# antonilo/unsupervised_detection

Hardware: NVIDIA H100
Metric: frame-pairs/sec adversarial train step 256x448 (higher is better)
Workload: dtype bf16

## Files before the change

unsupervised_detection_b200/csrc/conv_igemm.cu:

```cuda
#include "ptx.cuh"
#include "../../include/cis_b200.h"
#include "common.cuh"
#include <cuda.h>
#include <stdlib.h>
#include <string.h>


namespace cis {

#ifdef CIS_TRACE
__device__ unsigned long long* g_trace = nullptr;
__device__ int g_trace_cap = 0;
#define CIS_TRACE_AT(slot)                                                                                         \
  do {                                                                                                             \
    if (g_trace && blockIdx.x == 0 && blockIdx.y == 0 && blockIdx.z == 0 && (slot) < g_trace_cap) g_trace[(slot)] = clock64(); \
  } while (0)
#else
#define CIS_TRACE_AT(slot) ((void)0)
#endif

static constexpr int kBM = 128;
static constexpr int kBK = 64;
static constexpr int kAStage = kBM * 128;
static constexpr int kThreads = 256;
template <int BN, int NWG> struct HaloCfg {
  static_assert(NWG == 1 || (NWG == 2 && BN >= 64), "two MMA warpgroups only for BN >= 64");
  static constexpr int kMmaWarp = (NWG == 1 && BN >= 64) ? 8 : 4;
  static constexpr int kThreads = (kMmaWarp + 4 * NWG) * 32;
  static constexpr int kEpiWarps = NWG == 1 ? kMmaWarp : kThreads / 32;
  static constexpr int kEpiParts = NWG == 1 ? (BN >= 64 ? 2 : 1) : BN / 32;
  static constexpr int kMaxMT = (128 / BN) < 4 ? (128 / BN) : 4;
};
static constexpr int kMaxAccCols = 128;
static constexpr int kGProducers = 256;
static constexpr int kGThreads = 384;

struct SrcS {
  const __nv_bfloat16* ptr;
  int pitch, c_off, chunks, n_mod;
};


__device__ __forceinline__ void epi_chunk(const CisConv& p, float (&v)[16], const int cg, const size_t dpix) {
  if (p.bias) {
#pragma unroll
    for (int e = 0; e < 16; ++e) v[e] += __ldg(p.bias + cg + e);
  }
  if (p.add_pre && cg < p.out_ch) {
    const uint4* a = reinterpret_cast<const uint4*>(reinterpret_cast<const __nv_bfloat16*>(p.add_pre) + dpix * p.add_pre_pitch +
                                                    p.add_pre_coff + cg);
    const int nv = (p.out_ch - cg >= 16) ? 2 : 1;
    for (int h2 = 0; h2 < nv; ++h2) {
      const uint4 u = __ldg(a + h2);
      const uint32_t w4[4] = {u.x, u.y, u.z, u.w};
#pragma unroll
      for (int e = 0; e < 4; ++e) {
        v[h2 * 8 + 2 * e] += bf16lo(w4[e]);
        v[h2 * 8 + 2 * e + 1] += bf16hi(w4[e]);
      }
    }
  }
  if (p.addf_pre) {
    for (int e = 0; e < 16 && cg + e < p.outf_ch; ++e) v[e] += __ldg(p.addf_pre + dpix * p.addf_pitch + p.addf_coff + cg + e);
  }
// ... 183 lines not shown
#pragma unroll
    for (int h = 0; h < 4; ++h) t[h] = __ldcg(q0 + (size_t)z * zstride + h * kBM);
#pragma unroll
    for (int h = 0; h < 4; ++h) {
      v[4 * h] += t[h].x; v[4 * h + 1] += t[h].y; v[4 * h + 2] += t[h].z; v[4 * h + 3] += t[h].w;
    }
  }
}
template <int BN, typename DPIX>
__device__ __forceinline__ void cluster_reduce_rows(const CisConv& p, const uint32_t stage, const int S, const int rank, const int tid,
                                                    const int nthreads, const int cbase, DPIX dpix_of) {
  const int rpc = (kBM + S - 1) / S;
  const int r0 = rank * rpc, r1 = min(kBM, r0 + rpc);
  constexpr int G16 = BN / 16;
  for (int it = tid; it < (r1 - r0) * G16; it += nthreads) {
    const int row = r0 + it / G16, c0 = (it % G16) * 16;
    float v[16];
#pragma unroll
    for (int e = 0; e < 16; ++e) v[e] = 0.f;
    for (int q = 0; q < S; ++q) {
      const uint32_t base = dsmem_addr(stage, (uint32_t)q);
#pragma unroll
      for (int h = 0; h < 4; ++h) {
        const float4 t = dsmem_ld4(base + (uint32_t)(((c0 / 4 + h) * kBM + row) * 16));
        v[4 * h] += t.x; v[4 * h + 1] += t.y; v[4 * h + 2] += t.z; v[4 * h + 3] += t.w;
      }
    }
    bool valid;
    const size_t dpix = dpix_of(row, valid);
    if (valid) epi_chunk(p, v, cbase + c0, dpix);
  }
}

template <int BN>
struct FwdCfg {
  static constexpr int kStages = (BN == 128) ? 3 : 4;
  static constexpr int kLag = kStages - 2;
  static constexpr int kBStage = BN * 128;
  static constexpr int kSmem = kStages * (kAStage + kBStage) + 1024;
  static_assert(kStages * (kAStage + kBStage) >= kBM * BN * 4, "the accumulator tile reuses the operand ring");
};

template <int BN>
__global__ void __launch_bounds__(kGThreads) conv_igemm_kernel(const __grid_constant__ CisConv p) {
  using Cfg = FwdCfg<BN>;
  constexpr int S = Cfg::kStages;
  constexpr int kMmaWarp = kGProducers / 32;
  extern __shared__ uint8_t smem_raw[];
  __shared__ uint64_t bars[2 * S + 1];
  __shared__ int s_dh[CIS_MAX_TAPS], s_dw[CIS_MAX_TAPS];
  __shared__ SrcS s_src[CIS_MAX_SRC];

  const uint32_t tile_base = (smem_u32(smem_raw) + 1023u) & ~1023u;
  const uint32_t a_base = tile_base;
  const uint32_t b_base = tile_base + S * kAStage;
  const uint32_t bar_full = smem_u32(&bars[0]);
  const uint32_t bar_empty = smem_u32(&bars[S]);
  const uint32_t bar_accum = smem_u32(&bars[2 * S]);

  const int tid = threadIdx.x;
  const int warp = tid >> 5, lane = tid & 31;
  const int M = p.N * p.OH * p.OW;
  const int m_chunks = [&] {
    int s = 0;
    for (int i = 0; i < p.nsrc; ++i) s += p.src[i].chunks;
    return s;
  }();
  const int nkb_all = p.K_pad / kBK;
  const int nsplit = p.splits > 1 ? p.splits : 1;
  const int kper = (nkb_all + nsplit - 1) / nsplit;
  const int kb_lo = blockIdx.z * kper;
  const int nkb = min(kper, nkb_all - kb_lo);
  const int ny = blockIdx.y;
  __shared__ __align__(16) float s_bias[BN];
  pdl_launch_dependents();

  if (tid < p.ntaps) {
    s_dh[tid] = p.dh[tid];
    s_dw[tid] = p.dw[tid];
  }
  if (tid < p.nsrc) {
    s_src[tid].ptr = reinterpret_cast<const __nv_bfloat16*>(p.src[tid].ptr);
    s_src[tid].pitch = p.src[tid].pitch;
    s_src[tid].c_off = p.src[tid].c_off;
    s_src[tid].chunks = p.src[tid].chunks;
    s_src[tid].n_mod = p.src[tid].n_mod;
  }
  if (tid == kMmaWarp * 32) {
    for (int s = 0; s < S; ++s) {
      mbar_init(bar_full + 8 * s, kGProducers);
      mbar_init(bar_empty + 8 * s, 1);
    }
    mbar_init(bar_accum, 128);
    fence_mbar_init();
  }
  pdl_wait();
  if (tid < BN) s_bias[tid] = p.bias ? p.bias[ny * BN + tid] : 0.f;
  __syncthreads();
  if (tid == 0) CIS_TRACE_AT(0);

  if (warp < kMmaWarp) {
    const int j = tid & 7;
    const int rl = tid >> 3;
    const uint32_t sw_off = (uint32_t)((j ^ (rl & 7)) << 4);
    int hb[4], wb[4], pre[4], prem[4];
    int nm0 = 0;
    for (int i = 0; i < p.nsrc; ++i)
      if (p.src[i].n_mod > 0 && nm0 == 0) nm0 = p.src[i].n_mod;
#pragma unroll
    for (int i = 0; i < 4; ++i) {
      const int g = blockIdx.x * kBM + rl + 32 * i;
      if (g < M) {
        const int ow = g % p.OW;
        const int t = g / p.OW;
        const int oh = t % p.OH;
        const int n = t / p.OH;
        hb[i] = oh * p.sh;
        wb[i] = ow * p.sw;
        pre[i] = (n * p.H + hb[i]) * p.W + wb[i];
        prem[i] = ((nm0 ? n % nm0 : n) * p.H + hb[i]) * p.W + wb[i];
      } else {
        hb[i] = -(1 << 20);
        wb[i] = 0;
        pre[i] = prem[i] = 0;
      }
    }
    const __nv_bfloat16* wrow = reinterpret_cast<const __nv_bfloat16*>(p.wpack) + (size_t)(ny * BN + rl) * p.K_pad + j * 8;
    const int adv_t = 8 / m_chunks, adv_c = 8 - adv_t * m_chunks;
    int t = (kb_lo * 8 + j) / m_chunks, c = (kb_lo * 8 + j) - t * m_chunks;

    for (int kb = 0; kb < nkb; ++kb) {
      const int s = kb % S;
      const uint32_t ph = (uint32_t)((kb / S) & 1);
      mbar_wait(bar_empty + 8 * s, ph ^ 1u);
      const bool kvalid = t < p.ntaps;
      const int tt = kvalid ? t : 0;
      int si = 0, cs = c;
// ... 20 lines not shown
        }
        cp_async16(a_dst + i * 32 * 128, ok ? (const void*)(spc + (size_t)pix * pitch) : (const void*)sp, ok ? 16u : 0u);
      }
      t += adv_t;
      c += adv_c;
      if (c >= m_chunks) {
        c -= m_chunks;
        ++t;
      }
      const uint32_t b_dst = b_base + s * Cfg::kBStage + rl * 128 + sw_off;
      if constexpr (BN >= 32) {
#pragma unroll
        for (int i = 0; i < BN / 32; ++i) cp_async16(b_dst + i * 32 * 128, wrow + (size_t)i * 32 * p.K_pad + (kb_lo + kb) * kBK, 16u);
      } else {
        if (rl < BN) cp_async16(b_dst, wrow + (kb_lo + kb) * kBK, 16u);
      }
      cp_async_commit();
      if (kb >= Cfg::kLag) {
        cp_async_wait<Cfg::kLag>();
        fence_proxy_async();
        mbar_arrive(bar_full + 8 * ((kb - Cfg::kLag) % S));
      }
    }
#pragma unroll
    for (int i = Cfg::kLag - 1; i >= 0; --i) {
      if (nkb - 1 - i < 0) continue;
      if (i == 3) cp_async_wait<3>();
      else if (i == 2) cp_async_wait<2>();
      else if (i == 1) cp_async_wait<1>();
      else cp_async_wait<0>();
      fence_proxy_async();
      mbar_arrive(bar_full + 8 * ((nkb - 1 - i) % S));
    }

    mbar_wait(bar_accum, 0);
    if (tid == 0) CIS_TRACE_AT(2);
    const int qtr = warp & 3, half = warp >> 2;
    const int row = qtr * 32 + lane;
    const int g = blockIdx.x * kBM + row;
    const bool valid = g < M;
    size_t dpix = 0;
    if (valid) {
      const int ow = g % p.OW;
      const int t = g / p.OW;
      const int oh = t % p.OH;
      const int n = t / p.OH;
      dpix = (size_t)(n * p.DH + oh * p.osh + p.oa) * p.DW + ow * p.osw + p.ob;
    }
    const uint32_t t_row = tile_base + (uint32_t)row * 16;
    const int cbase = ny * BN;
    constexpr int kHalf = BN >= 32 ? BN / 2 : BN;
    const int c_lo = half * kHalf, c_hi = (BN >= 32 || half == 0) ? c_lo + kHalf : c_lo;
    if (nsplit > 1 && p.sk_cluster) {
    } else if (nsplit > 1) {
      const int tile_id = blockIdx.x * gridDim.y + ny;
      float* tile0 = p.sk_scratch + (size_t)tile_id * nsplit * kBM * BN;
      splitk_store_partial<BN>(tile0 + (size_t)blockIdx.z * kBM * BN, t_row, row, c_lo, c_hi);
    } else {
      epi_cols<BN>(p, t_row, cbase, dpix, valid, s_bias, c_lo, c_hi);
    }
  } else {
    const int wtid = tid - kMmaWarp * 32;
    float acc[BN];
    const uint32_t dhi = desc_hi(1024);
    constexpr uint32_t a_half = (8 * 1024) >> 4;
    for (int kb = 0; kb < nkb; ++kb) {
      const int s = kb % S;
      mbar_wait(bar_full + 8 * s, (uint32_t)((kb / S) & 1));
      if (wtid == 0) CIS_TRACE_AT(8 + 2 * kb);
      const uint32_t alo = desc_lo(a_base + s * kAStage, 16), blo = desc_lo(b_base + s * Cfg::kBStage, 16);
      wg_fence();
#pragma unroll
      for (int k = 0; k < kBK / 16; ++k) mma128<BN, 0, 0>(acc, alo + 2 * k, dhi, blo + 2 * k, dhi, a_half, (uint32_t)((kb | k) != 0));
      wg_commit();
      wg_wait<1>();
      if (wtid == 0 && kb > 0) mbar_arrive(bar_empty + 8 * ((kb - 1) % S));
      if (wtid == 0) CIS_TRACE_AT(9 + 2 * kb);
    }
    wg_wait<0>();
    acc_store<BN>(acc, tile_base, wtid);
    mbar_arrive(bar_accum);
  }
  if (nsplit > 1 && p.sk_cluster) {
    cluster_sync_all();
    if (warp < kMmaWarp) {
      const int cbase = ny * BN;
      cluster_reduce_rows<BN>(p, tile_base, nsplit, (int)cluster_ctarank(), tid, kGProducers, cbase, [&](int row, bool& valid) -> size_t {
        const int g = blockIdx.x * kBM + row;
        valid = g < M;
        if (!valid) return 0;
        const int ow = g % p.OW;
        const int t = g / p.OW;
        const int oh = t % p.OH;
        const int n = t / p.OH;
        return (size_t)(n * p.DH + oh * p.osh + p.oa) * p.DW + ow * p.osw + p.ob;
      });
    }
    cluster_sync_all();
  }
  if (tid == 0) CIS_TRACE_AT(3);
}


static constexpr int kHaloMaxBStages = 8;
struct HaloMaps {
  CUtensorMap m[CIS_MAX_SRC * 4];
  CUtensorMap w;
  int wrow;
  int16_t wk[2 * CIS_MAX_TAPS];
};
__device__ __forceinline__ void wrow_load(const HaloMaps& maps, const uint32_t dst, const uint32_t bar, const int s0, const int ns, const int n0,
                                          const int BN) {
  for (int s = 0; s < ns; ++s)
// ... 56 lines not shown
    while (ph < p.nph - 1 && t >= p.ph_tap[ph + 1]) ++ph;
  return (uint32_t)(ph * (p.thin / 8)) * plane16 + (uint32_t)(p.dh[t] * Wh + p.dw[t]);
}
__device__ __forceinline__ uint32_t halo_step_off(const CisConv& p, const int t0, const int nt, const int s, const int Wh, const uint32_t plane16) {
  if (!p.thin) return (uint32_t)((p.dh[t0 + s] * Wh + p.dw[t0 + s]) * 8);
  const int ta = p.thin == 8 ? 2 * s : s;
  const uint32_t o0 = halo_tap_off(p, t0 + ta, Wh, plane16);
  if (p.thin == 16) return o0 | (plane16 << 16);
  const uint32_t o1 = ta + 1 < nt ? halo_tap_off(p, t0 + ta + 1, Wh, plane16) : o0;
  return o0 | ((o1 - o0) << 16);
}
template <typename Src>
__device__ __forceinline__ void thin_halo_load(const CisConv& p, const Src* src, const HaloMaps& maps, const uint32_t dst, const uint32_t bar,
                                               const int HP, const int x0, const int y0, const int n) {
  const int nph = p.nph > 1 ? p.nph : 1, npl = p.thin / 8, pb16 = thin_plane_bytes(HP);
  int nld = 0;
  for (int ph = 0; ph < nph; ++ph) nld += nph == 1 || p.ph_tap[ph + 1] > p.ph_tap[ph];
  mbar_expect_tx(bar, (uint32_t)(nld * npl * HP * 16));
  for (int ph = 0; ph < nph; ++ph) {
    if (nph > 1 && p.ph_tap[ph + 1] == p.ph_tap[ph]) continue;
    for (int q = 0; q < npl; ++q) {
      int cq = q, sq = 0;
      while (sq < p.nsrc - 1 && cq >= src[sq].chunks) {
        cq -= src[sq].chunks;
        ++sq;
      }
      const int nm = src[sq].n_mod;
      tma_load_4d(dst + (ph * npl + q) * pb16, &maps.m[sq * nph + ph], bar, cq * 8, x0, y0, nm ? (n % nm) : n);
    }
  }
}

template <int BN, int NWG>
__global__ void __launch_bounds__(HaloCfg<BN, NWG>::kThreads, 1) conv_halo_kernel(const __grid_constant__ CisConv p, const int halo_stage_bytes, const int BS, const int NHS,
                                                        const __grid_constant__ HaloMaps maps, const int use_tma, const int G) {
  using Cfg = HaloCfg<BN, NWG>;
  constexpr int kBStage = BN * 128;
  constexpr int kHMmaWarp_ = Cfg::kMmaWarp, kHThreads_ = Cfg::kThreads;
  extern __shared__ uint8_t smem_raw[];
  __shared__ uint64_t bars[2 * 2 + 2 * kHaloMaxBStages + 1];
  __shared__ uint32_t s_aoff[CIS_MAX_TAPS];
  __shared__ SrcS s_src[CIS_MAX_SRC];

  const int tid = threadIdx.x, warp = tid >> 5, lane = tid & 31;
  const int MT = p.MT, MTC = NWG * MT, d = p.dil;
  const int nph = p.nph > 1 ? p.nph : 1;
  const int Wh = 8 + p.ex, Hh = 16 * MTC + p.ey, HP = Wh * Hh;
  const int thin = p.thin;
  const int nhph = thin ? 1 : nph;
  const uint32_t wstep = thin ? BN * 32 : kBStage;
  const uint32_t stage_bytes = (uint32_t)G * wstep;
  const uint32_t tile_base = (smem_u32(smem_raw) + 1023u) & ~1023u;
  const uint32_t h_base = tile_base;
  const uint32_t b_base = tile_base + NHS * halo_stage_bytes;
  int* pixtab = reinterpret_cast<int*>(smem_raw + (b_base + BS * stage_bytes - smem_u32(smem_raw)));
  const uint32_t bar_hfull = smem_u32(&bars[0]), bar_hempty = smem_u32(&bars[2]);
  const uint32_t bar_bfull = smem_u32(&bars[4]), bar_bempty = smem_u32(&bars[4 + kHaloMaxBStages]);
  const uint32_t bar_accum = smem_u32(&bars[4 + 2 * kHaloMaxBStages]);

  const bool grouped = p.nsub > 1;
  const int tap0 = grouped ? p.sub[blockIdx.z].tap0 : 0, ntaps = grouped ? p.sub[blockIdx.z].ntaps : p.ntaps;
  const int nst = halo_nsteps(thin, ntaps);
  const int hoy = grouped ? p.sub[blockIdx.z].hoy : p.hoy, hox = grouped ? p.sub[blockIdx.z].hox : p.hox;
  const int OHs = grouped ? p.sub[blockIdx.z].OH : p.OH, OWs = grouped ? p.sub[blockIdx.z].OW : p.OW;
  const int oa = grouped ? p.sub[blockIdx.z].oa : p.oa, ob = grouped ? p.sub[blockIdx.z].ob : p.ob;
  const void* const wpack = grouped ? p.sub[blockIdx.z].wpack : p.wpack;
  const int Hp0 = (OHs + d - 1) / d, Wp0 = (OWs + d - 1) / d;
// ... 19 lines not shown
  if (tid < nst) s_aoff[tid] = halo_step_off(p, tap0, ntaps, tid, Wh, (uint32_t)thin_plane_bytes(HP) >> 4);
  if (tid < p.nsrc) {
    s_src[tid].ptr = reinterpret_cast<const __nv_bfloat16*>(p.src[tid].ptr);
    s_src[tid].pitch = p.src[tid].pitch;
    s_src[tid].c_off = p.src[tid].c_off;
    s_src[tid].chunks = p.src[tid].chunks;
    s_src[tid].n_mod = p.src[tid].n_mod;
  }
  for (int q = tid; q < (use_tma ? 0 : HP); q += kHThreads_) {
    const int hy = q / Wh, hx = q - hy * Wh;
    const int gy = ty * 16 * MTC + hy + hoy, gx = tx * 8 + hx + hox;
    const int y = pa + d * gy, x = pb + d * gx;
    pixtab[q] = (gy >= 0 && gx >= 0 && y < p.H && x < p.W) ? (y * p.W + x) : -1;
  }
  if (tid == kHMmaWarp_ * 32) {
    for (int s = 0; s < 2; ++s) {
      mbar_init(bar_hfull + 8 * s, use_tma ? 1 : 96);
      mbar_init(bar_hempty + 8 * s, NWG);
    }
    for (int s = 0; s < BS; ++s) {
      mbar_init(bar_bfull + 8 * s, 1);
      mbar_init(bar_bempty + 8 * s, NWG);
    }
    mbar_init(bar_accum, 128 * NWG);
    fence_mbar_init();
  }
  if (use_tma && tid < p.nsrc) tma_prefetch_desc(&maps.m[tid]);
  pdl_wait();
  if (tid < BN) s_bias[tid] = p.bias ? p.bias[ny * BN + tid] : 0.f;
  __syncthreads();
  if (tid == 0) CIS_TRACE_AT(0);

  if (warp < kHMmaWarp_) {
   if (warp < 4) {
    if (use_tma) {
      if (tid == 0) {
        int hcount = 0;
        for (int vc = 0; vc < nchunks * nhph; ++vc) {
          const int cc = vc / nhph, ph = vc - cc * nhph;
          if (nhph > 1 && p.ph_tap[ph + 1] == p.ph_tap[ph]) continue;
          const int hs = hcount % NHS;
          mbar_wait(bar_hempty + 8 * hs, (uint32_t)(((hcount / NHS) & 1) ^ 1));
          ++hcount;
          int c = (cc_lo + cc) * 8, si = 0;
          while (si < p.nsrc - 1 && c >= s_src[si].chunks) {
            c -= s_src[si].chunks;
            ++si;
          }
          const int nmod = s_src[si].n_mod;
          if (thin) {
            thin_halo_load(p, s_src, maps, h_base + hs * halo_stage_bytes, bar_hfull + 8 * hs, HP, tx * 8 + hox, ty * 16 * MTC + hoy, n);
            continue;
          }
          mbar_expect_tx(bar_hfull + 8 * hs, (uint32_t)(HP * 128));
          tma_load_4d(h_base + hs * halo_stage_bytes, &maps.m[si * nph + ph], bar_hfull + 8 * hs, c * 8, pb + d * (tx * 8 + hox),
                      pa + d * (ty * 16 * MTC + hoy), nmod ? (n % nmod) : n);
        }
      }
      __syncwarp();
    } else if (warp != 2) {
      const int hid = warp == 3 ? tid - 32 : tid;
      const int j = hid & 7, pl = hid >> 3;
      for (int cc = 0; cc < nchunks; ++cc) {
        const int hs = cc % NHS;
        mbar_wait(bar_hempty + 8 * hs, (uint32_t)(((cc / NHS) & 1) ^ 1));
        const int rem = m_chunks - (cc_lo + cc) * 8;
        const int nk16 = rem >= 8 ? 4 : (rem + 1) / 2;
// ... 29 lines not shown
        } else if (cc >= 1) {
          cp_async_wait<1>();
          fence_proxy_async();
          mbar_arrive(bar_hfull + 8 * ((cc - 1) % NHS));
        }
      }
      if (NHS > 1) {
        cp_async_wait<0>();
        fence_proxy_async();
        mbar_arrive(bar_hfull + 8 * ((nchunks - 1) % NHS));
      }
    }
    if (tid == 64) {
      const uint8_t* wt = reinterpret_cast<const uint8_t*>(wpack) + ((size_t)ny * nchunks_all + cc_lo) * nst * wstep;
      int bs = 0;
      uint32_t bph = 1;
      for (int vc = 0; vc < nchunks * nhph; ++vc) {
        const int cc = vc / nhph, ph = vc - cc * nhph;
        const int tlo = nhph > 1 ? p.ph_tap[ph] : 0, thi = nhph > 1 ? p.ph_tap[ph + 1] : nst;
        for (int t0 = tlo; t0 < thi; t0 += G) {
          const uint32_t bytes = (uint32_t)min(G, thi - t0) * wstep;
          mbar_wait(bar_bempty + 8 * bs, bph);
          mbar_expect_tx(bar_bfull + 8 * bs, bytes);
          if (maps.wrow) wrow_load(maps, b_base + bs * stage_bytes, bar_bfull + 8 * bs, t0, min(G, thi - t0), ny * BN, BN);
          else bulk_g2s(b_base + bs * stage_bytes, wt + (size_t)(cc * nst + t0) * wstep, bytes, bar_bfull + 8 * bs);
          if (++bs == BS) {
            bs = 0;
            bph ^= 1u;
          }
        }
      }
    }
    __syncwarp();
   }

  } else {
    const int wg = NWG > 1 ? (warp - kHMmaWarp_) >> 2 : 0;
    const int wtid = tid - (kHMmaWarp_ + 4 * wg) * 32;
    constexpr int MTM = Cfg::kMaxMT;
    float acc[MTM][BN];
    const uint32_t pix = thin ? 16u : 128u;
    const uint32_t ahi = thin ? desc_hi_ns((uint32_t)Wh * pix) : desc_hi((uint32_t)Wh * pix);
    const uint32_t bhi = thin ? desc_hi_ns(maps.wrow ? 128u : 256u) : desc_hi(1024), b_lbo = maps.wrow ? BN * 16u : thin ? 128u : 16u;
    const uint32_t a_mstep = (16u * Wh * pix) >> 4;
    const uint32_t a_half = (8u * Wh * pix) >> 4;
    const uint32_t a_wg = (uint32_t)(wg * MT) * a_mstep;
    int bs = 0, hs = 0, it = 0;
    uint32_t bph = 0, hph = 0;
    bool any = false;
    for (int vc = 0; vc < nchunks * nhph; ++vc) {
      const int cc = vc / nhph, ph = vc - cc * nhph;
      const int tlo = nhph > 1 ? p.ph_tap[ph] : 0, thi = nhph > 1 ? p.ph_tap[ph + 1] : nst;
      if (thi == tlo) continue;
      const int rem = m_chunks - (cc_lo + cc) * 8;
      const int nk16 = rem >= 8 ? 4 : (rem + 1) / 2;
      mbar_wait(bar_hfull + 8 * hs, hph);
      if (vc == 0 && wtid == 0 && wg == 0) CIS_TRACE_AT(1);
      const uint32_t hlo = desc_lo(h_base + hs * halo_stage_bytes, thin ? 0 : 16) + a_wg;
      for (int t0 = tlo; t0 < thi; t0 += G, ++it) {
        const int gt = min(G, thi - t0);
        mbar_wait(bar_bfull + 8 * bs, bph);
        if (wtid == 0 && wg == 0) CIS_TRACE_AT(8 + 2 * it);
        const uint32_t blo = desc_lo(b_base + bs * stage_bytes, b_lbo);
        halo_issue_any<BN, MTM>(nk16, acc, hlo, blo, s_aoff + t0, gt, MT, ahi, bhi, a_mstep, a_half, wstep >> 4, !any);
        if (wtid == 0) {
          mbar_arrive(bar_bempty + 8 * bs);
          if (t0 + G >= thi) mbar_arrive(bar_hempty + 8 * hs);
          if (wg == 0) CIS_TRACE_AT(9 + 2 * it);
        }
        any = true;
        if (++bs == BS) {
          bs = 0;
          bph ^= 1u;
        }
      }
      if (++hs == NHS) {
        hs = 0;
        hph ^= 1u;
      }
    }
    if constexpr (NWG > 1) asm volatile("bar.sync 1, %0;" ::"n"(128 * NWG) : "memory");
#pragma unroll
    for (int m = 0; m < MTM; ++m)
      if (m < MT) acc_store<BN>(acc[m], tile_base + (uint32_t)((wg * MT + m) * BN) * kAccColBytes, wtid);
    mbar_arrive(bar_accum);
  }

  if (warp < Cfg::kEpiWarps) {
    mbar_wait(bar_accum, 0);
    if (tid == 0) CIS_TRACE_AT(2);
    constexpr int kParts = Cfg::kEpiParts, kCols = BN / kParts, kUnits = 4 * kParts;
    const int cbase = ny * BN;
    const int tile_id = blockIdx.x * gridDim.y + ny;
    if (!(nsplit > 1 && p.sk_cluster)) {
#pragma unroll 1
      for (int u = warp; u < MTC * kUnits; u += Cfg::kEpiWarps) {
        const int m = u / kUnits, r = (u & 3) * 32 + lane, c_lo = ((u >> 2) % kParts) * kCols, c_hi = c_lo + kCols;
        const uint32_t t_row = tile_base + (uint32_t)(m * BN) * kAccColBytes + (uint32_t)r * 16;
        if (nsplit > 1) {
          splitk_store_partial<BN>(p.sk_scratch + (((size_t)tile_id * MTC + m) * nsplit + blockIdx.z) * kBM * BN, t_row, r, c_lo, c_hi);
        } else {
          const int gy = ty * 16 * MTC + 16 * m + (r >> 3), gx = tx * 8 + (r & 7);
          const int oy = pa + d * gy, ox = pb + d * gx;
          const bool valid = oy < OHs && ox < OWs;
          const size_t dpix = valid ? ((size_t)(n * p.DH + oy * p.osh + oa) * p.DW + ox * p.osw + ob) : 0;
          epi_cols<BN>(p, t_row, cbase, dpix, valid, s_bias, c_lo, c_hi);
        }
      }
    }
  }
  if (nsplit > 1 && p.sk_cluster) {
    cluster_sync_all();
    if (warp < 4) {
      const int cbase = ny * BN;
      for (int m = 0; m < MTC; ++m)
        cluster_reduce_rows<BN>(p, tile_base + (uint32_t)m * (kBM * BN * 4), nsplit, (int)cluster_ctarank(), tid, 128, cbase,
                                [&](int row, bool& valid) -> size_t {
// ... 699 lines not shown
  cfg.numAttrs = pdl_enabled() ? 1 : 0;
  return cudaLaunchKernelEx(&cfg, kern, KArgs(args)...);
}

template <typename... KArgs, typename... Args>
static cudaError_t launch_pdl_zcluster(void (*kern)(KArgs...), dim3 grid, dim3 block, size_t smem, cudaStream_t st, int cz, Args... args) {
  cudaLaunchConfig_t cfg;
  memset(&cfg, 0, sizeof(cfg));
  cfg.gridDim = grid;
  cfg.blockDim = block;
  cfg.dynamicSmemBytes = smem;
  cfg.stream = st;
  cudaLaunchAttribute attr[2];
  attr[0].id = cudaLaunchAttributeClusterDimension;
  attr[0].val.clusterDim.x = 1;
  attr[0].val.clusterDim.y = 1;
  attr[0].val.clusterDim.z = cz;
  attr[1].id = cudaLaunchAttributeProgrammaticStreamSerialization;
  attr[1].val.programmaticStreamSerializationAllowed = 1;
  cfg.attrs = attr;
  cfg.numAttrs = pdl_enabled() ? 2 : 1;
  return cudaLaunchKernelEx(&cfg, kern, KArgs(args)...);
}

template <int BN>
static cudaError_t launch_splitk_finish(const CisConv* d, dim3 main_grid, cudaStream_t st) {
  constexpr int G = BN / 16;
  constexpr int kBlock = (128 * G < 256) ? 128 * G : 256;
  constexpr int kSub = 128 * G / kBlock;
  const int mt = d->halo ? d->MT * (d->nwg > 1 ? d->nwg : 1) : 1;
  return launch_pdl(splitk_finish_kernel<BN>, dim3(main_grid.x, main_grid.y, mt * kSub), dim3(kBlock), 0, st, *d);
}

template <int BN>
static int launch_fwd(const CisConv* d, cudaStream_t st) {
  using Cfg = FwdCfg<BN>;
  static bool attr_set = false;
  if (!attr_set) {
    cudaError_t e = cudaFuncSetAttribute(conv_igemm_kernel<BN>, cudaFuncAttributeMaxDynamicSharedMemorySize, Cfg::kSmem);
    if (e != cudaSuccess) return cis_set_cuda_error(e, "cudaFuncSetAttribute(conv_igemm)");
    attr_set = true;
  }
  const int M = d->N * d->OH * d->OW;
  int splits = d->splits > 1 ? d->splits : 1;
  if (splits > 1) {
    const int nkb = d->K_pad / kBK, per = (nkb + splits - 1) / splits;
    if ((!d->sk_scratch && !d->sk_cluster) || d->sk_counters || (splits - 1) * per >= nkb || (d->sk_cluster && splits > 8))
      return cis_set_error(CIS_ERR_BAD_ARG, "cis_conv_igemm: bad split-K setup");
  }
  dim3 grid((M + kBM - 1) / kBM, d->n_tiles, splits);
  cudaError_t le = (splits > 1 && d->sk_cluster)
                       ? launch_pdl_zcluster(conv_igemm_kernel<BN>, grid, dim3(kGThreads), Cfg::kSmem, st, splits, *d)
                       : launch_pdl(conv_igemm_kernel<BN>, grid, dim3(kGThreads), Cfg::kSmem, st, *d);
  if (le != cudaSuccess) return cis_set_cuda_error(le, "launch(conv_igemm)");
  if (splits > 1 && !d->sk_cluster) {
    le = launch_splitk_finish<BN>(d, grid, st);
    if (le != cudaSuccess) return cis_set_cuda_error(le, "launch(splitk_finish)");
  }
  return cis_check_launch("conv_igemm");
}


typedef CUresult (*EncodeTiledFn)(CUtensorMap*, CUtensorMapDataType, cuuint32_t, void*, const cuuint64_t*, const cuuint64_t*, const cuuint32_t*,
                                  const cuuint32_t*, CUtensorMapInterleave, CUtensorMapSwizzle, CUtensorMapL2promotion, CUtensorMapFloatOOBfill);
static EncodeTiledFn get_encode_tiled() {
  static EncodeTiledFn fn = nullptr;
  static bool tried = false;
  if (!tried) {
    tried = true;
    void* p = nullptr;
    cudaDriverEntryPointQueryResult q;
    if (cudaGetDriverEntryPoint("cuTensorMapEncodeTiled", &p, cudaEnableDefault, &q) == cudaSuccess && q == cudaDriverEntryPointSuccess)
      fn = (EncodeTiledFn)p;
  }
  return fn;
}
static bool encode_src_map(CUtensorMap* m, const CisSrc& s, int N, int H, int W, int bw, int bh, int step = 1, int py = 0, int px = 0,
                           int estride = 1, int bc = 64, CUtensorMapSwizzle swz = CU_TENSOR_MAP_SWIZZLE_128B) {
  EncodeTiledFn enc = get_encode_tiled();
  if (!enc) return false;
  const int nb = s.n_mod > 0 ? s.n_mod : N;
  const int Hq = (H - py + step - 1) / step, Wq = (W - px + step - 1) / step;
  if (Hq < 1 || Wq < 1) return false;
  cuuint64_t dims[4] = {(cuuint64_t)s.chunks * 8, (cuuint64_t)Wq, (cuuint64_t)Hq, (cuuint64_t)nb};
  cuuint64_t strides[3] = {(cuuint64_t)step * s.pitch * 2, (cuuint64_t)step * W * s.pitch * 2, (cuuint64_t)H * W * s.pitch * 2};
  cuuint32_t box[4] = {(cuuint32_t)bc, (cuuint32_t)(bw * estride), (cuuint32_t)(bh * estride), 1};
  cuuint32_t es[4] = {1, (cuuint32_t)estride, (cuuint32_t)estride, 1};
  void* base = (void*)((const char*)s.ptr + ((size_t)(py * W + px) * s.pitch + (size_t)s.c_off) * 2);
  return enc(m, CU_TENSOR_MAP_DATA_TYPE_BFLOAT16, 4, base, dims, strides, box, es, CU_TENSOR_MAP_INTERLEAVE_NONE, swz,
             CU_TENSOR_MAP_L2_PROMOTION_L2_128B, CU_TENSOR_MAP_FLOAT_OOB_FILL_NONE) == CUDA_SUCCESS;
}

#ifdef CIS_TRACE
extern "C" int cis_trace_set(unsigned long long* buf, int cap) {
  cudaError_t e = cudaMemcpyToSymbol(cis::g_trace, &buf, sizeof(buf));
  if (e == cudaSuccess) e = cudaMemcpyToSymbol(cis::g_trace_cap, &cap, sizeof(cap));
  return e == cudaSuccess ? CIS_OK : cis_set_cuda_error(e, "cis_trace_set");
}
#endif

static int g_persist_mode = -1;
extern "C" int cis_set_persist_mode(int mode) {
  g_persist_mode = mode;
  return CIS_OK;
}

template <int BN, int NWG>
static int launch_halo(const CisConv* d, cudaStream_t st, const int16_t* wk = nullptr) {
  const int MTC = d->MT * NWG;
  const int Wh = 8 + d->ex, Hh = 16 * MTC + d->ey, HP = Wh * Hh;
  const int thin = d->thin;
  const int nph = d->nph > 1 ? d->nph : 1;
  const int halo_stage = ((thin ? nph * (thin / 8) * thin_plane_bytes(HP) : HP * 128) + 1023) & ~1023;
  int chunks = 0;
  for (int i = 0; i < d->nsrc; ++i) chunks += d->src[i].chunks;
  if (thin && ((thin != 8 && thin != 16) || chunks * 8 != thin || d->dil != 1))
    return cis_set_error(CIS_ERR_BAD_ARG, "cis_conv_igemm(halo): the compact format needs 8 or 16 undilated input channels");
  const int nchunks = (chunks + 7) / 8;
  const int nsub = d->nsub > 1 ? d->nsub : 1;
  const int nsp = (nsub == 1 && d->splits > 1) ? d->splits : 1;
  const int cper = (nchunks + nsp - 1) / nsp;
  const int nhs = cper > 1 ? 2 : 1;
  const int dd = d->dil;
  int tiles = 0, ntaps_max = d->ntaps;
  if (nsub > 1) {
    if (nsub > 4 || dd != 1 || d->splits > 1 || d->nph > 1) return cis_set_error(CIS_ERR_BAD_ARG, "cis_conv_igemm(halo): bad grouped launch");
    ntaps_max = 0;
    int tsum = 0;
    for (int i = 0; i < nsub; ++i) {
      const int t = ((d->sub[i].OW + 7) / 8) * ((d->sub[i].OH + 16 * MTC - 1) / (16 * MTC));
      if (t > tiles) tiles = t;
      if (d->sub[i].ntaps > ntaps_max) ntaps_max = d->sub[i].ntaps;
      if (d->sub[i].ntaps < 1 || d->sub[i].tap0 != tsum || !d->sub[i].wpack) return cis_set_error(CIS_ERR_BAD_ARG, "cis_conv_igemm(halo): bad sub-problem");
      tsum += d->sub[i].ntaps;
    }
    if (tsum != d->ntaps) return cis_set_error(CIS_ERR_BAD_ARG, "cis_conv_igemm(halo): sub-problem taps must add up to ntaps");
  } else {
    const int Hp0 = (d->OH + dd - 1) / dd, Wp0 = (d->OW + dd - 1) / dd;
    tiles = ((Wp0 + 7) / 8) * ((Hp0 + 16 * MTC - 1) / (16 * MTC));
  }
  if (thin == 8) {
    for (int i = 0; i < nsub; ++i) {
      const int t0 = nsub > 1 ? d->sub[i].tap0 : 0, nt = nsub > 1 ? d->sub[i].ntaps : d->ntaps;
      for (int t = t0 + 1; t < t0 + nt; ++t)
        if (!(nph > 1 && (t == d->ph_tap[1] || t == d->ph_tap[2] || t == d->ph_tap[3])) &&
            d->dh[t] * (8 + d->ex) + d->dw[t] < d->dh[t - 1] * (8 + d->ex) + d->dw[t - 1])
          return cis_set_error(CIS_ERR_BAD_ARG, "cis_conv_igemm(halo): compact 8-channel taps must be listed in increasing halo offset");
    }
  }
  const int nst_max = halo_nsteps(thin, ntaps_max);
  const long ncta_all = (long)tiles * dd * dd * d->N * d->n_tiles * nsp * nsub;
  static const int g_env = getenv("CIS_HALO_G") ? atoi(getenv("CIS_HALO_G")) : 0;
  static const int stage_kb = getenv("CIS_HALO_STAGE_KB") ? atoi(getenv("CIS_HALO_STAGE_KB")) : 48;
  const int kB = thin ? BN * 32 : BN * 128;
  int G = g_env > 0 ? g_env : (stage_kb * 1024) / kB;
  if (G < 1) G = 1;
  if (G > nst_max) G = nst_max;
  const int fixed = nhs * halo_stage + HP * 4 + 1024;
  static const int lim_small_kb = getenv("CIS_HALO_SMALL_KB") ? atoi(getenv("CIS_HALO_SMALL_KB")) : 226;
  static const int lim_kb_wide = getenv("CIS_HALO_LIMIT_KB") ? atoi(getenv("CIS_HALO_LIMIT_KB")) : 113;
  static const int lim_kb_thin = getenv("CIS_HALO_LIMIT_THIN_KB") ? atoi(getenv("CIS_HALO_LIMIT_THIN_KB")) : 113;
  const int lim_kb = BN <= 32 ? lim_kb_thin : lim_kb_wide;
  const int nsm = cis_num_sms();
  int limit = (ncta_all > nsm && fixed + 2 * kB <= lim_kb * 1024) ? lim_kb * 1024 : 226 * 1024;
  if (ncta_all <= nsm && fixed + 2 * kB <= lim_small_kb * 1024) limit = lim_small_kb * 1024;
  while (G > 1 && fixed + 2 * G * kB > limit) --G;
  const int groups = cper * ((nsub > 1 ? 1 : (nst_max + G - 1) / G));
  int BS = (limit - fixed) / (G * kB);
  if (BS > (ncta_all > nsm ? 4 : kHaloMaxBStages)) BS = ncta_all > nsm ? 4 : kHaloMaxBStages;
  if (BS > groups) BS = groups;
  if (BS < 1) return cis_set_error(CIS_ERR_UNSUPPORTED, "cis_conv_igemm(halo): tile does not fit shared memory");
  int smem = fixed + BS * G * kB;
  if (smem < MTC * kBM * BN * 4 + 1024) smem = MTC * kBM * BN * 4 + 1024;
  if (smem > 226 * 1024) return cis_set_error(CIS_ERR_UNSUPPORTED, "cis_conv_igemm(halo): accumulator tiles do not fit shared memory");
  static int attr_smem = 0;
  if (smem > attr_smem) {
    cudaError_t e = cudaFuncSetAttribute(conv_halo_kernel<BN, NWG>, cudaFuncAttributeMaxDynamicSharedMemorySize, smem);
    if (e != cudaSuccess) return cis_set_cuda_error(e, "cudaFuncSetAttribute(conv_halo)");
    attr_smem = smem;
  }

  int splits = d->splits > 1 ? d->splits : 1;
  if (splits > 1) {
    const int per = (nchunks + splits - 1) / splits;
    if ((!d->sk_scratch && !d->sk_cluster) || d->sk_counters || (splits - 1) * per >= nchunks || (d->sk_cluster && splits > 8))
      return cis_set_error(CIS_ERR_BAD_ARG, "cis_conv_igemm(halo): bad split-K setup");
  }
  dim3 grid(tiles * dd * dd * d->N, d->n_tiles, nsub > 1 ? nsub : splits);
  HaloMaps maps;
  static const int dil_tma = getenv("CIS_DIL_TMA") ? atoi(getenv("CIS_DIL_TMA")) : 1;
  int use_tma = ((d->dil == 1 || dil_tma) && Wh * d->dil <= 256 && Hh * d->dil <= 256) ? 1 : 0;
  for (int i = 0; use_tma && !thin && i < d->nsrc - 1; ++i)
    if (d->src[i].chunks % 8) use_tma = 0;
  for (int i = 0; use_tma && i < d->nsrc; ++i) {
    if (((uintptr_t)d->src[i].ptr + (size_t)d->src[i].c_off * 2) % 16) use_tma = 0;
    for (int ph = 0; use_tma && ph < nph; ++ph)
      if (!(thin ? encode_src_map(&maps.m[i * nph + ph], d->src[i], d->N, d->H, d->W, Wh, Hh, nph > 1 ? 2 : 1, ph >> 1, ph & 1, 1, 8,
// ... 304 lines not shown
```

unsupervised_detection_b200/csrc/ptx.cuh:

```cuda
#pragma once
#include <cuda_runtime.h>
#include <cuda_bf16.h>
#include <stdint.h>

namespace cis {

__device__ __forceinline__ uint32_t smem_u32(const void* p) {
  return static_cast<uint32_t>(__cvta_generic_to_shared(p));
}

__device__ __forceinline__ void mbar_init(uint32_t bar, uint32_t count) {
  asm volatile("mbarrier.init.shared::cta.b64 [%0], %1;" ::"r"(bar), "r"(count) : "memory");
}
__device__ __forceinline__ void fence_mbar_init() {
  asm volatile("fence.mbarrier_init.release.cluster;" ::: "memory");
}
__device__ __forceinline__ void mbar_arrive(uint32_t bar) {
  asm volatile("{\n\t.reg .b64 st;\n\tmbarrier.arrive.shared::cta.b64 st, [%0];\n\t}" ::"r"(bar) : "memory");
}
__device__ __forceinline__ void mbar_expect_tx(uint32_t bar, uint32_t bytes) {
  asm volatile("{\n\t.reg .b64 st;\n\tmbarrier.arrive.expect_tx.shared::cta.b64 st, [%0], %1;\n\t}" ::"r"(bar), "r"(bytes)
               : "memory");
}
__device__ __forceinline__ bool mbar_try_wait(uint32_t bar, uint32_t parity) {
// ... 36 lines not shown
      "cp.async.bulk.tensor.4d.shared::cluster.global.mbarrier::complete_tx::bytes [%0], [%1, {%3, %4, %5, %6}], [%2];" ::"r"(dst),
      "l"(tmap), "r"(bar), "r"(c0), "r"(c1), "r"(c2), "r"(c3)
      : "memory");
}
__device__ __forceinline__ void bulk_g2s(uint32_t dst, const void* src, uint32_t bytes, uint32_t bar) {
  asm volatile("cp.async.bulk.shared::cluster.global.mbarrier::complete_tx::bytes [%0], [%1], %2, [%3];" ::"r"(dst), "l"(src), "r"(bytes),
               "r"(bar)
               : "memory");
}
__device__ __forceinline__ uint32_t cluster_ctarank() {
  uint32_t r;
  asm volatile("mov.u32 %0, %%cluster_ctarank;" : "=r"(r));
  return r;
}
__device__ __forceinline__ void cluster_sync_all() {
  asm volatile("barrier.cluster.arrive.release.aligned;\n\tbarrier.cluster.wait.acquire.aligned;" ::: "memory");
}
__device__ __forceinline__ uint32_t dsmem_addr(uint32_t saddr, uint32_t rank) {
  uint32_t r;
  asm volatile("mapa.shared::cluster.u32 %0, %1, %2;" : "=r"(r) : "r"(saddr), "r"(rank));
  return r;
}
__device__ __forceinline__ float4 dsmem_ld4(uint32_t caddr) {
  float4 v;
  asm volatile("ld.shared::cluster.v4.f32 {%0, %1, %2, %3}, [%4];" : "=f"(v.x), "=f"(v.y), "=f"(v.z), "=f"(v.w) : "r"(caddr) : "memory");
  return v;
}
__device__ __forceinline__ void tma_prefetch_desc(const void* tmap) {
  asm volatile("prefetch.tensormap [%0];" ::"l"(tmap) : "memory");
}

__device__ __forceinline__ void pdl_launch_dependents() { asm volatile("griddepcontrol.launch_dependents;" ::: "memory"); }
__device__ __forceinline__ void pdl_wait() { asm volatile("griddepcontrol.wait;" ::: "memory"); }

__device__ __forceinline__ void wg_fence() { asm volatile("wgmma.fence.sync.aligned;" ::: "memory"); }
__device__ __forceinline__ void wg_commit() { asm volatile("wgmma.commit_group.sync.aligned;" ::: "memory"); }
template <int N>
__device__ __forceinline__ void wg_wait() {
  asm volatile("wgmma.wait_group.sync.aligned %0;" ::"n"(N) : "memory");
}

template <int N, int TA, int TB> struct Wgmma;
template <int TA, int TB> struct Wgmma<16, TA, TB> {
  static __device__ __forceinline__ void mma(float (&d)[8], uint64_t da, uint64_t db, uint32_t scale_d) {
    asm volatile(
        "{\n\t.reg .pred p;\n\tsetp.ne.b32 p, %10, 0;\n\t"
        "wgmma.mma_async.sync.aligned.m64n16k16.f32.bf16.bf16 {%0,%1,%2,%3,%4,%5,%6,%7}, %8, %9, p, 1, 1, %11, %12;\n\t}"
        : "+f"(d[0]), "+f"(d[1]), "+f"(d[2]), "+f"(d[3]), "+f"(d[4]), "+f"(d[5]), "+f"(d[6]), "+f"(d[7])
        : "l"(da), "l"(db), "r"(scale_d), "n"(TA), "n"(TB));
  }
};
template <int TA, int TB> struct Wgmma<32, TA, TB> {
  static __device__ __forceinline__ void mma(float (&d)[16], uint64_t da, uint64_t db, uint32_t scale_d) {
    asm volatile(
        "{\n\t.reg .pred p;\n\tsetp.ne.b32 p, %18, 0;\n\t"
        "wgmma.mma_async.sync.aligned.m64n32k16.f32.bf16.bf16 {%0,%1,%2,%3,%4,%5,%6,%7,%8,%9,%10,%11,%12,%13,%14,%15}, %16, %17, p, 1, 1, %19, %20;\n\t}"
        : "+f"(d[0]), "+f"(d[1]), "+f"(d[2]), "+f"(d[3]), "+f"(d[4]), "+f"(d[5]), "+f"(d[6]), "+f"(d[7]), "+f"(d[8]), "+f"(d[9]), "+f"(d[10]), "+f"(d[11]), "+f"(d[12]), "+f"(d[13]), "+f"(d[14]), "+f"(d[15])
        : "l"(da), "l"(db), "r"(scale_d), "n"(TA), "n"(TB));
  }
};
template <int TA, int TB> struct Wgmma<64, TA, TB> {
  static __device__ __forceinline__ void mma(float (&d)[32], uint64_t da, uint64_t db, uint32_t scale_d) {
    asm volatile(
        "{\n\t.reg .pred p;\n\tsetp.ne.b32 p, %34, 0;\n\t"
        "wgmma.mma_async.sync.aligned.m64n64k16.f32.bf16.bf16 {%0,%1,%2,%3,%4,%5,%6,%7,%8,%9,%10,%11,%12,%13,%14,%15,%16,%17,%18,%19,%20,%21,%22,%23,%24,%25,%26,%27,%28,%29,%30,%31}, %32, %33, p, 1, 1, %35, %36;\n\t}"
        : "+f"(d[0]), "+f"(d[1]), "+f"(d[2]), "+f"(d[3]), "+f"(d[4]), "+f"(d[5]), "+f"(d[6]), "+f"(d[7]), "+f"(d[8]), "+f"(d[9]), "+f"(d[10]), "+f"(d[11]), "+f"(d[12]), "+f"(d[13]), "+f"(d[14]), "+f"(d[15]), "+f"(d[16]), "+f"(d[17]), "+f"(d[18]), "+f"(d[19]), "+f"(d[20]), "+f"(d[21]), "+f"(d[22]), "+f"(d[23]), "+f"(d[24]), "+f"(d[25]), "+f"(d[26]), "+f"(d[27]), "+f"(d[28]), "+f"(d[29]), "+f"(d[30]), "+f"(d[31])
// ... 63 lines not shown
```

Measured before the change: 662.0.

## Run two CTAs per SM with warp-specialized register reallocation in conv kernels

Adds setmaxnreg-based register rebalancing between producer and MMA warpgroups so the implicit-GEMM forward kernel (BN=64) and the single-warpgroup halo kernel can fit two CTAs per SM. The halo kernel drops from 8 to 4 producer warps, and the smem budget is derived from the per-SM limit so pairs fit. Launch picks one CTA per SM when the grid fits in a single wave. The aim is better latency hiding through higher occupancy, at the cost of fewer producer threads, tighter register limits (possible spills) and smaller pipelines per CTA.

Result: faster. 695.1, median of 6 (+5.0%).

```diff
diff --git a/unsupervised_detection_b200/csrc/conv_igemm.cu b/unsupervised_detection_b200/csrc/conv_igemm.cu
--- a/unsupervised_detection_b200/csrc/conv_igemm.cu
+++ b/unsupervised_detection_b200/csrc/conv_igemm.cu
@@ -25,11 +25,17 @@
 static constexpr int kThreads = 256;
 template <int BN, int NWG> struct HaloCfg {
   static_assert(NWG == 1 || (NWG == 2 && BN >= 64), "two MMA warpgroups only for BN >= 64");
-  static constexpr int kMmaWarp = (NWG == 1 && BN >= 64) ? 8 : 4;
+  static constexpr int kMmaWarp = 4;
   static constexpr int kThreads = (kMmaWarp + 4 * NWG) * 32;
-  static constexpr int kEpiWarps = NWG == 1 ? kMmaWarp : kThreads / 32;
+  static constexpr int kEpiWarps = (NWG == 1 && BN < 64) ? kMmaWarp : kThreads / 32;
   static constexpr int kEpiParts = NWG == 1 ? (BN >= 64 ? 2 : 1) : BN / 32;
   static constexpr int kMaxMT = (128 / BN) < 4 ? (128 / BN) : 4;
+  static constexpr int kCtasPerSm = NWG == 1 ? 2 : 1;
+  static constexpr int kLaunchRegs = (65536 / (kCtasPerSm * kThreads)) & ~7;
+  static constexpr int kProdRegs = (NWG == 1 && BN >= 32) ? 88 : 0;
+  static constexpr int kMmaRegs = (NWG == 1 && BN >= 32) ? 168 : 0;
+  static_assert(kProdRegs == 0 || 128 * (kProdRegs + NWG * kMmaRegs) <= kThreads * kLaunchRegs,
+                "setmaxnreg.inc would wait for registers the CTA does not own");
 };
 static constexpr int kMaxAccCols = 128;
 static constexpr int kGProducers = 256;
@@ -279,18 +285,24 @@
   }
 }
 
-template <int BN>
+template <int BN, int CPS>
 struct FwdCfg {
   static constexpr int kStages = (BN == 128) ? 3 : 4;
   static constexpr int kLag = kStages - 2;
   static constexpr int kBStage = BN * 128;
   static constexpr int kSmem = kStages * (kAStage + kBStage) + 1024;
   static_assert(kStages * (kAStage + kBStage) >= kBM * BN * 4, "the accumulator tile reuses the operand ring");
+  static_assert(CPS == 1 || BN <= 64, "128 accumulator columns do not fit two CTAs per SM");
+  static constexpr int kLaunchRegs = (65536 / (CPS * kGThreads)) & ~7;
+  static constexpr int kProdRegs = (BN == 64 && CPS == 2) ? 72 : 0;
+  static constexpr int kMmaRegs = (BN == 64 && CPS == 2) ? 96 : 0;
+  static_assert(kProdRegs == 0 || 128 * (kProdRegs * kGProducers / 128 + kMmaRegs) <= kGThreads * kLaunchRegs,
+                "setmaxnreg.inc would wait for registers the CTA does not own");
 };
 
-template <int BN>
-__global__ void __launch_bounds__(kGThreads) conv_igemm_kernel(const __grid_constant__ CisConv p) {
-  using Cfg = FwdCfg<BN>;
+template <int BN, int CPS>
+__global__ void __launch_bounds__(kGThreads, CPS == 1 ? 0 : CPS) conv_igemm_kernel(const __grid_constant__ CisConv p) {
+  using Cfg = FwdCfg<BN, CPS>;
   constexpr int S = Cfg::kStages;
   constexpr int kMmaWarp = kGProducers / 32;
   extern __shared__ uint8_t smem_raw[];
@@ -350,6 +362,7 @@
     const int j = tid & 7;
     const int rl = tid >> 3;
     const uint32_t sw_off = (uint32_t)((j ^ (rl & 7)) << 4);
+    if constexpr (Cfg::kProdRegs > 0) setmaxnreg_dec<Cfg::kProdRegs>();
     int hb[4], wb[4], pre[4], prem[4];
     int nm0 = 0;
     for (int i = 0; i < p.nsrc; ++i)
@@ -436,6 +449,10 @@
       fence_proxy_async();
       mbar_arrive(bar_full + 8 * ((nkb - 1 - i) % S));
     }
+    if constexpr (Cfg::kProdRegs > 0) {
+      named_bar_sync<2, kGProducers>();
+      setmaxnreg_inc<Cfg::kLaunchRegs>();
+    }
 
     mbar_wait(bar_accum, 0);
     if (tid == 0) CIS_TRACE_AT(2);
@@ -464,6 +481,7 @@
       epi_cols<BN>(p, t_row, cbase, dpix, valid, s_bias, c_lo, c_hi);
     }
   } else {
+    if constexpr (Cfg::kMmaRegs > 0) setmaxnreg_inc<Cfg::kMmaRegs>();
     const int wtid = tid - kMmaWarp * 32;
     float acc[BN];
     const uint32_t dhi = desc_hi(1024);
@@ -483,6 +501,10 @@
     }
     wg_wait<0>();
     acc_store<BN>(acc, tile_base, wtid);
+    if constexpr (Cfg::kMmaRegs > 0) {
+      named_bar_sync<3, 128>();
+      setmaxnreg_dec<Cfg::kLaunchRegs>();
+    }
     mbar_arrive(bar_accum);
   }
   if (nsplit > 1 && p.sk_cluster) {
@@ -605,7 +627,7 @@
 }
 
 template <int BN, int NWG>
-__global__ void __launch_bounds__(HaloCfg<BN, NWG>::kThreads, 1) conv_halo_kernel(const __grid_constant__ CisConv p, const int halo_stage_bytes, const int BS, const int NHS,
+__global__ void __launch_bounds__(HaloCfg<BN, NWG>::kThreads, HaloCfg<BN, NWG>::kCtasPerSm) conv_halo_kernel(const __grid_constant__ CisConv p, const int halo_stage_bytes, const int BS, const int NHS,
                                                         const __grid_constant__ HaloMaps maps, const int use_tma, const int G) {
   using Cfg = HaloCfg<BN, NWG>;
   constexpr int kBStage = BN * 128;
@@ -691,7 +713,7 @@
   if (tid == 0) CIS_TRACE_AT(0);
 
   if (warp < kHMmaWarp_) {
-   if (warp < 4) {
+    if constexpr (Cfg::kProdRegs > 0) setmaxnreg_dec<Cfg::kProdRegs>();
     if (use_tma) {
       if (tid == 0) {
         int hcount = 0;
@@ -787,9 +809,12 @@
       }
     }
     __syncwarp();
-   }
-
+    if constexpr (Cfg::kProdRegs > 0) {
+      named_bar_sync<2, 128>();
+      setmaxnreg_inc<Cfg::kLaunchRegs>();
+    }
   } else {
+    if constexpr (Cfg::kMmaRegs > 0) setmaxnreg_inc<Cfg::kMmaRegs>();
     const int wg = NWG > 1 ? (warp - kHMmaWarp_) >> 2 : 0;
     const int wtid = tid - (kHMmaWarp_ + 4 * wg) * 32;
     constexpr int MTM = Cfg::kMaxMT;
@@ -838,6 +863,10 @@
 #pragma unroll
     for (int m = 0; m < MTM; ++m)
       if (m < MT) acc_store<BN>(acc[m], tile_base + (uint32_t)((wg * MT + m) * BN) * kAccColBytes, wtid);
+    if constexpr (Cfg::kMmaRegs > 0) {
+      named_bar_sync<3, 128>();
+      setmaxnreg_dec<Cfg::kLaunchRegs>();
+    }
     mbar_arrive(bar_accum);
   }
 
@@ -1603,12 +1632,12 @@
   return launch_pdl(splitk_finish_kernel<BN>, dim3(main_grid.x, main_grid.y, mt * kSub), dim3(kBlock), 0, st, *d);
 }
 
-template <int BN>
-static int launch_fwd(const CisConv* d, cudaStream_t st) {
-  using Cfg = FwdCfg<BN>;
+template <int BN, int CPS>
+static int launch_fwd_cps(const CisConv* d, cudaStream_t st) {
+  using Cfg = FwdCfg<BN, CPS>;
   static bool attr_set = false;
   if (!attr_set) {
-    cudaError_t e = cudaFuncSetAttribute(conv_igemm_kernel<BN>, cudaFuncAttributeMaxDynamicSharedMemorySize, Cfg::kSmem);
+    cudaError_t e = cudaFuncSetAttribute(conv_igemm_kernel<BN, CPS>, cudaFuncAttributeMaxDynamicSharedMemorySize, Cfg::kSmem);
     if (e != cudaSuccess) return cis_set_cuda_error(e, "cudaFuncSetAttribute(conv_igemm)");
     attr_set = true;
   }
@@ -1621,14 +1650,22 @@
   }
   dim3 grid((M + kBM - 1) / kBM, d->n_tiles, splits);
   cudaError_t le = (splits > 1 && d->sk_cluster)
-                       ? launch_pdl_zcluster(conv_igemm_kernel<BN>, grid, dim3(kGThreads), Cfg::kSmem, st, splits, *d)
-                       : launch_pdl(conv_igemm_kernel<BN>, grid, dim3(kGThreads), Cfg::kSmem, st, *d);
+                       ? launch_pdl_zcluster(conv_igemm_kernel<BN, CPS>, grid, dim3(kGThreads), Cfg::kSmem, st, splits, *d)
+                       : launch_pdl(conv_igemm_kernel<BN, CPS>, grid, dim3(kGThreads), Cfg::kSmem, st, *d);
   if (le != cudaSuccess) return cis_set_cuda_error(le, "launch(conv_igemm)");
   if (splits > 1 && !d->sk_cluster) {
     le = launch_splitk_finish<BN>(d, grid, st);
     if (le != cudaSuccess) return cis_set_cuda_error(le, "launch(splitk_finish)");
   }
   return cis_check_launch("conv_igemm");
+}
+template <int BN>
+static int launch_fwd(const CisConv* d, cudaStream_t st) {
+  const long ncta = (long)((d->N * d->OH * d->OW + kBM - 1) / kBM) * d->n_tiles * (d->splits > 1 ? d->splits : 1);
+  if constexpr (BN == 64) {
+    if (ncta <= cis_num_sms()) return launch_fwd_cps<BN, 1>(d, st);
+  }
+  return launch_fwd_cps<BN, BN == 128 ? 1 : 2>(d, st);
 }
 
 
@@ -1674,6 +1711,17 @@
 extern "C" int cis_set_persist_mode(int mode) {
   g_persist_mode = mode;
   return CIS_OK;
+}
+
+template <typename K>
+static int pair_smem_limit(K kernel) {
+  int dev = 0, per_sm = 0, reserved = 0;
+  cudaFuncAttributes fa;
+  if (cudaGetDevice(&dev) != cudaSuccess || cudaDeviceGetAttribute(&per_sm, cudaDevAttrMaxSharedMemoryPerMultiprocessor, dev) != cudaSuccess ||
+      cudaDeviceGetAttribute(&reserved, cudaDevAttrReservedSharedMemoryPerBlock, dev) != cudaSuccess ||
+      cudaFuncGetAttributes(&fa, kernel) != cudaSuccess)
+    return 112 * 1024;
+  return (per_sm / 2 - reserved - (int)fa.sharedSizeBytes) & ~1023;
 }
 
 template <int BN, int NWG>
@@ -1728,12 +1776,14 @@
   if (G < 1) G = 1;
   if (G > nst_max) G = nst_max;
   const int fixed = nhs * halo_stage + HP * 4 + 1024;
+  static const int lim_pair = HaloCfg<BN, NWG>::kCtasPerSm == 2 ? pair_smem_limit(conv_halo_kernel<BN, NWG>) : 113 * 1024;
   static const int lim_small_kb = getenv("CIS_HALO_SMALL_KB") ? atoi(getenv("CIS_HALO_SMALL_KB")) : 226;
-  static const int lim_kb_wide = getenv("CIS_HALO_LIMIT_KB") ? atoi(getenv("CIS_HALO_LIMIT_KB")) : 113;
-  static const int lim_kb_thin = getenv("CIS_HALO_LIMIT_THIN_KB") ? atoi(getenv("CIS_HALO_LIMIT_THIN_KB")) : 113;
+  static const int lim_kb_wide = getenv("CIS_HALO_LIMIT_KB") ? atoi(getenv("CIS_HALO_LIMIT_KB")) : 0;
+  static const int lim_kb_thin = getenv("CIS_HALO_LIMIT_THIN_KB") ? atoi(getenv("CIS_HALO_LIMIT_THIN_KB")) : 0;
   const int lim_kb = BN <= 32 ? lim_kb_thin : lim_kb_wide;
+  const int lim = lim_kb > 0 ? lim_kb * 1024 : lim_pair;
   const int nsm = cis_num_sms();
-  int limit = (ncta_all > nsm && fixed + 2 * kB <= lim_kb * 1024) ? lim_kb * 1024 : 226 * 1024;
+  int limit = (ncta_all > nsm && fixed + 2 * kB <= lim) ? lim : 226 * 1024;
   if (ncta_all <= nsm && fixed + 2 * kB <= lim_small_kb * 1024) limit = lim_small_kb * 1024;
   while (G > 1 && fixed + 2 * G * kB > limit) --G;
   const int groups = cper * ((nsub > 1 ? 1 : (nst_max + G - 1) / G));
diff --git a/unsupervised_detection_b200/csrc/ptx.cuh b/unsupervised_detection_b200/csrc/ptx.cuh
--- a/unsupervised_detection_b200/csrc/ptx.cuh
+++ b/unsupervised_detection_b200/csrc/ptx.cuh
@@ -92,6 +92,19 @@
 
 __device__ __forceinline__ void pdl_launch_dependents() { asm volatile("griddepcontrol.launch_dependents;" ::: "memory"); }
 __device__ __forceinline__ void pdl_wait() { asm volatile("griddepcontrol.wait;" ::: "memory"); }
+
+template <int ID, int N>
+__device__ __forceinline__ void named_bar_sync() {
+  asm volatile("bar.sync %0, %1;" ::"n"(ID), "n"(N) : "memory");
+}
+template <int R>
+__device__ __forceinline__ void setmaxnreg_inc() {
+  asm volatile("setmaxnreg.inc.sync.aligned.u32 %0;" ::"n"(R));
+}
+template <int R>
+__device__ __forceinline__ void setmaxnreg_dec() {
+  asm volatile("setmaxnreg.dec.sync.aligned.u32 %0;" ::"n"(R));
+}
 
 __device__ __forceinline__ void wg_fence() { asm volatile("wgmma.fence.sync.aligned;" ::: "memory"); }
 __device__ __forceinline__ void wg_commit() { asm volatile("wgmma.commit_group.sync.aligned;" ::: "memory"); }
```
